# fjall-rs/lsm-tree

Measured on AMD Instinct MI355X. Metric: device-resident data-block decode+encode GiB/s, 1 M × 4 KiB blocks, higher is better.
Workload: dtype u8; 1 GPU; BASELINE configs[1]/[2]: encode + decode round trip of 1 M x 4 KiB data blocks, device-resident; blocks_per_gpu=1048576, items_per_gpu=54525952, block_bytes_per_gpu=3953267212, restart_interval=16, key_len=16, val_len=64, parallelism=shard1 (independent block batches, no collective)

## Files before the change

### lsm-tree_amd/csrc/encode_group.hpp

```cpp
#pragma once

#include "encode_plan.hpp"

namespace lsmgpu {

struct GBlk {
  uint32_t it0, n;
  uint32_t img, plen;
  uint32_t recs, bin_len;
  uint32_t step, hash_w;
  uint32_t hash_base, u0;
  uint32_t nbk, spare;
};
static_assert(sizeof(GBlk) == 48, "GBlk");

#ifdef LSM_NO_WAVE_BLOCKS
constexpr bool kWaveBlocks = false;
#else
constexpr bool kWaveBlocks = true;
#endif
constexpr uint32_t kWKeys = 1024, kWVals = 4096, kWImg = 4496;
constexpr uint32_t kWItems = kWave;
constexpr uint32_t kWUnits = 5;
static_assert((kWImg - 1) / 1024 <= 4 && (kWImg - 1) / 1024 + 1 <= kWUnits,
              "full KiB units and the tail unit of a payload");
constexpr uint32_t kWDefer = 4;
static_assert(kWDefer >= 1 && kWDefer <= kWave / 4, "one lane quad per deferred block");
static_assert(kWDefer * kWUnits * 8 * 8 <= kWImg, "the kept contributions fit the free image at the flush");
struct WaveSlot {
  uint8_t keys[kWKeys + kGSlack];
  uint8_t vals[kWVals + kGSlack];
  uint8_t img[kWImg + kGSlack];
  uint64_t contrib[kWUnits * 8];
};
static_assert(offsetof(WaveSlot, vals) % 16 == 0 && offsetof(WaveSlot, img) % 16 == 0 && sizeof(WaveSlot) % 16 == 0,
              "stage DMA and 16-B copy-out alignment");
constexpr uint32_t kGroupBody = kGKeys + kGVals + kGImg + 3 * kGSlack + kGUnion + 2 * kGBlocks * (uint32_t)sizeof(GBlk);
constexpr uint32_t kWaveSlots = kGWaves * (uint32_t)sizeof(WaveSlot);
constexpr uint32_t kWavePad = kWaveSlots > kGroupBody ? kWaveSlots - kGroupBody : 16;

struct GroupLds {
  uint8_t keys[kGKeys + kGSlack];
  uint8_t vals[kGVals + kGSlack];
  uint8_t img[kGImg + kGSlack];
  uint32_t uni[kGUnion / 4];
  GBlk blk[2][kGBlocks];
  uint8_t wave_pad[kWavePad];
  LongSecret secret;
};
static_assert(offsetof(GroupLds, uni) - offsetof(GroupLds, vals) >= sizeof(PlanWaveLds), "plan LDS over the stage");
static_assert(offsetof(GroupLds, vals) % 16 == 0, "plan LDS alignment");
static_assert(kGRunFused * (sizeof(BlockPlan) + 8) + 16 <= kGUnion, "fused plan outputs in uni");
static_assert(offsetof(GroupLds, wave_pad) == kGroupBody, "GroupLds layout");
static_assert(kGWaves * sizeof(WaveSlot) <= offsetof(GroupLds, secret), "the wave slots lie over the group loop's LDS");
static_assert(sizeof(GroupLds) <= 40960, "four workgroups per CU");

__device__ __host__ __forceinline__ bool wave_fits(uint64_t n, uint64_t kspan, uint64_t vspan, uint64_t total) {
  return n >= 1 && n <= kWItems && kspan + 15 <= kWKeys && vspan + 15 <= kWVals && total + 15 <= kWImg;
}


__device__ __forceinline__ void lds_copy(uint8_t* dst, uint32_t d, const uint8_t* src, uint32_t s, uint32_t n,
                                         uint32_t rot, uint32_t done = 0) {
  if (!n) return;
  const uint32_t h = min(n, (4u - (d & 3u)) & 3u);
  uint32_t hb[3];
#pragma unroll
  for (uint32_t k = 0; k < 3; ++k)
    if (k < h) hb[k] = src[s + k];
#pragma unroll
  for (uint32_t k = 0; k < 3; ++k)
    if (k < h) dst[d + k] = (uint8_t)hb[k];
  if (n == h) return;
  const uint32_t d1 = d + h + 4 * done, e = d + n, body = ((e & ~3u) - d1) >> 2;
  const uint32_t sp = s + h + 4 * done, sh = sp & 3u;
  const uint32_t* s32 = reinterpret_cast<const uint32_t*>(src + (sp & ~3u));
  uint32_t* d32 = reinterpret_cast<uint32_t*>(dst + d1);
  uint32_t q = ((rot & 31u) * body) >> 5;
  constexpr uint32_t U = 4;
  const uint32_t w0 = body ? s32[0] : 0;
  uint32_t carry = body ? s32[q] : 0;
  for (uint32_t j0 = 0; j0 < body; j0 += U) {
    uint32_t hi[U], at[U];
#pragma unroll
    for (uint32_t t = 0; t < U; ++t) {
      uint32_t p = q + t;
      p = p >= body ? p - body : p;
      at[t] = p;
      if (j0 + t < body) hi[t] = s32[p + 1];
    }
#pragma unroll
    for (uint32_t t = 0; t < U; ++t) {
      if (j0 + t < body) {
        const uint32_t lo = t == 0 ? carry : (at[t] == 0 ? w0 : hi[t - 1]);
        d32[at[t]] = alignbyte(hi[t], lo, sh);
      }
    }
    q += U;
    q = q >= body ? q - body : q;
    carry = q == 0 ? w0 : hi[U - 1];
  }
  const uint32_t t0 = d1 + 4 * body;
  uint32_t tb[3];
#pragma unroll
  for (uint32_t k = 0; k < 3; ++k)
    if (t0 + k < e) tb[k] = src[s + (t0 + k - d)];
#pragma unroll
  for (uint32_t k = 0; k < 3; ++k)
    if (t0 + k < e) dst[t0 + k] = (uint8_t)tb[k];
}

#ifdef LSM_NO_UNIFORM_COPY
constexpr bool kUniformCopy = false;
#else
constexpr bool kUniformCopy = true;
#endif
constexpr uint32_t kUniformMin = 4;
__device__ __forceinline__ uint32_t lds_copy_uniform(uint8_t* dst, uint32_t d, const uint8_t* src, uint32_t s,
                                                     uint32_t n, bool has, uint32_t rot) {
  if (!kUniformCopy) return 0;
  const uint32_t h = min(n, (4u - (d & 3u)) & 3u);
  const uint32_t body = n > h ? (((d + n) & ~3u) - (d + h)) >> 2 : 0u;
  const uint32_t B = wave_min_u32(has ? body : 0xFFFFFFFFu);
  if (B < kUniformMin || B == 0xFFFFFFFFu) return 0;
  if (has) {
    const uint8_t* sb = src + ((s + h) & ~3u);
    uint8_t* db = dst + d + h;
    const uint32_t sh = (s + h) & 3u, B4 = 4 * B;
    auto ld = [&](uint32_t x) { return *reinterpret_cast<const uint32_t*>(sb + x); };
    auto st = [&](uint32_t x, uint32_t v) { *reinterpret_cast<uint32_t*>(db + x) = v; };
    constexpr uint32_t U = kUniformMin;
    uint32_t x = (((rot & 31u) * B) >> 5) * 4;
    const uint32_t w0 = ld(0);
    uint32_t carry = ld(x);
    for (uint32_t j = 0; j < B; j += U) {
      uint32_t at[U], hi[U];
#pragma unroll
      for (uint32_t t = 0; t < U; ++t) {
        const uint32_t y = x + 4 * t;
        at[t] = t == 0 ? x : min(y, y - B4);
        hi[t] = ld(at[t] + 4);
      }
#pragma unroll
      for (uint32_t t = 0; t < U; ++t) {
        const uint32_t lo = at[t] == 0 ? w0 : (t == 0 ? carry : hi[t - 1]);
        st(at[t], alignbyte(hi[t], lo, sh));
      }
      carry = hi[U - 1];
      x += 4 * U;
      x = min(x, x - B4);
    }
    if (body > B) {
      st(B4, alignbyte(ld(B4 + 4), ld(B4), sh));
      return B + 1;
    }
  }
  return B;
}

__device__ __forceinline__ uint32_t lds_put_leb(uint8_t* dst, uint32_t pos, uint64_t v) {
  while (v >= 0x80) {
    dst[pos++] = (uint8_t)(v | 0x80);
    v >>= 7;
  }
  dst[pos++] = (uint8_t)v;
  return pos;
}

template <bool kIndex>
__device__ __forceinline__ uint32_t put_record_header(uint8_t* img, uint32_t pos, const uint8_t* keys, uint32_t kst,
                                                      const ItemMeta& m, bool head, uint32_t from, uint32_t rot) {
  if (kIndex) {
    img[pos++] = 0;
    pos = lds_put_leb(img, pos, m.vo);
    pos = lds_put_leb(img, pos, m.vl);
    pos = lds_put_leb(img, pos, m.seq);
    pos = lds_put_leb(img, pos, m.klen);
    lds_copy(img, pos, keys, kst, m.klen, rot);
  } else {
    img[pos++] = (uint8_t)m.vt;
    pos = lds_put_leb(img, pos, m.seq);
    if (!head) pos = lds_put_leb(img, pos, m.sh);
    pos = lds_put_leb(img, pos, m.klen - from);
    lds_copy(img, pos, keys, kst + from, m.klen - from, rot);
    pos += m.klen - from;
    if (!is_tombstone(m.vt)) pos = lds_put_leb(img, pos, m.vl);
  }
  return pos;
}

__device__ __forceinline__ void put_bin_entry(uint8_t* img, uint32_t bp, const uint32_t& step, uint32_t roff) {
  for (uint32_t q = 0; q < step; ++q) img[bp + q] = (uint8_t)(roff >> (8 * q));
}

__device__ __forceinline__ void group_barrier() {
  __builtin_amdgcn_fence(__ATOMIC_RELEASE, "workgroup", "local");
  __builtin_amdgcn_s_barrier();
  __builtin_amdgcn_fence(__ATOMIC_ACQUIRE, "workgroup", "local");
}

__device__ __forceinline__ void group_barrier_lds() {
  asm volatile("s_waitcnt lgkmcnt(0)\n\ts_barrier" ::: "memory");
}

#ifdef LSM_DIAG
#define ENC_PHASE(i)                                 \
  if (P.diag & kDiagGroupPhases) {                              \
    const uint64_t t_ = __builtin_amdgcn_s_memtime(); \
    ph_acc[i] += (uint32_t)(t_ - t_last);            \
    t_last = t_;                                     \
  }
#else
#define ENC_PHASE(i)
#endif

constexpr uint64_t kLbAgg = 1ULL << 62, kLbIncl = 2ULL << 62, kLbPoison = 1ULL << 61, kLbVal = kLbPoison - 1;
constexpr uint64_t kLookbackTicks = 10000000;

__device__ __forceinline__ uint64_t lb_load(const uint64_t* p) {
  return __hip_atomic_load(p, __ATOMIC_RELAXED, __HIP_MEMORY_SCOPE_AGENT);
}
__device__ __forceinline__ void lb_store(uint64_t* p, uint64_t v) {
  __hip_atomic_store(p, v, __ATOMIC_RELAXED, __HIP_MEMORY_SCOPE_AGENT);
}

__device__ __noinline__ uint64_t run_lookback(uint64_t* lb, uint32_t run, uint64_t agg, uint32_t diag, bool& poisoned) {
  const int lane = threadIdx.x & (kWave - 1);
  if (lane == 0) lb_store(lb + run, (run == 0 ? kLbIncl : kLbAgg) | agg);
  uint64_t excl = 0;
  bool poison = false;
  if (run != 0) {
    int64_t top = (int64_t)run - 1;
    uint64_t t0 = __builtin_amdgcn_s_memrealtime();
    for (;;) {
      const int64_t idx = top - lane;
      const uint64_t v = idx >= 0 ? lb_load(lb + idx) : kLbIncl;
      const uint64_t incl_m = __ballot((v >> 62) == 2), ready_m = __ballot((v >> 62) != 0);
      const uint32_t stop = incl_m ? (uint32_t)__builtin_ctzll(incl_m) : 64u;
      const uint64_t need = stop >= 63 ? ~0ULL : (2ULL << stop) - 1;
      if ((ready_m & need) == need && !(kDiagBuild && (diag & kDiagLookbackGiveUp))) {
        const bool mine = (uint32_t)lane <= stop;
        poison = poison || __ballot(mine && (v & kLbPoison)) != 0;
        excl += wave_bcast_u64(wave_incl_scan_u64(mine ? (v & kLbVal) : 0), kWave - 1);
        if (stop < 64) break;
        top -= 64;
        t0 = __builtin_amdgcn_s_memrealtime();
        continue;
      }
      if (__builtin_amdgcn_s_memrealtime() - t0 > kLookbackTicks || (kDiagBuild && (diag & kDiagLookbackGiveUp))) {
        poison = true;
        break;
      }
      __builtin_amdgcn_s_sleep(1);
    }
    if (lane == 0) lb_store(lb + run, kLbIncl | (poison ? kLbPoison : 0) | ((excl + agg) & kLbVal));
  }
  poisoned = poison;
  return excl;
}

__device__ __forceinline__ uint32_t lane_u32(uint32_t v, uint32_t l) {
  return (uint32_t)__shfl((int)v, (int)min(l, 63u));
}
__device__ __forceinline__ uint64_t lane_u64(uint64_t v, uint32_t l) { return wave_shfl_u64(v, (int)min(l, 63u)); }
__device__ __forceinline__ uint32_t rl32(uint32_t v, uint32_t l) {
  return (uint32_t)__builtin_amdgcn_readlane((int)v, (int)min(l, 63u));
}
__device__ __forceinline__ uint64_t rl64(uint64_t v, uint32_t l) {
  const int q = (int)min(l, 63u);
  return (uint64_t)(uint32_t)__builtin_amdgcn_readlane((int)(uint32_t)v, q) |
         ((uint64_t)(uint32_t)__builtin_amdgcn_readlane((int)(uint32_t)(v >> 32), q) << 32);
}
__device__ __forceinline__ uint32_t tpi_shift(uint32_t n) {
  return n <= kGThreads / 4 ? 2u : n <= kGThreads / 2 ? 1u : 0u;
}
template <bool kIndex, class Raw>
__device__ __forceinline__ ItemMeta cook_vetted(const Raw& r) {
  bool bad = false;
  return cook_item<kIndex>(r, bad);
}

template <bool kIndex, bool kHash, bool kPlanBkt, int kOW, bool kFused = false>
__global__ __launch_bounds__(kGThreads) __attribute__((amdgpu_waves_per_eu(4))) void encode_group_kernel(EncodeParams P) {
  static_assert(!kFused || (!kIndex && !kHash), "the fused plan is for data blocks without a hash index");
  __shared__ GroupLds L;
  const uint32_t tid = threadIdx.x;
  const uint32_t wave = __builtin_amdgcn_readfirstlane(tid / kWave);
  const int lane = tid & (kWave - 1);
  constexpr uint32_t kRun = kFused ? kGRunFused : kGRun;
  const uint32_t b_begin = blockIdx.x * kRun;
  const uint32_t b_end = min(b_begin + kRun, P.n_blocks);
  const uint32_t ri = kIndex ? 1 : P.ri;
  constexpr bool index = kIndex;
  if (tid < sizeof(LongSecret) / 8)
    reinterpret_cast<uint64_t*>(&L.secret)[tid] = reinterpret_cast<const uint64_t*>(&kLongSecret)[tid];
  const uint32_t rb = b_begin + lane;
  const bool in_run = rb <= b_end;
  const uint32_t r_start = in_run ? P.starts[rb] : 0;
  uint64_t r_off, r_ks, r_vs;
  BlockPlan r_plan;
  bool run_ok = true;
  if (kFused) {
    BlockPlan* const fplan = reinterpret_cast<BlockPlan*>(L.uni);
    uint64_t* const fsize = reinterpret_cast<uint64_t*>(L.uni) + 2 * kRun;
    uint64_t* const fbase = fsize + kRun;
    plan_wave_run<false, kOW, true>(P, b_begin, b_end - b_begin, *reinterpret_cast<PlanWaveLds*>(L.vals), fplan,
                                    fsize);
    __syncthreads();
    r_plan = rb < b_end ? fplan[lane] : BlockPlan{0, 0, 0, 0};
    const uint64_t sz = rb < b_end ? fsize[lane] : 0;
    const uint64_t incl = wave_incl_scan_u64(sz);
    if (wave == 0) {
      bool poisoned;
      const uint64_t base = run_lookback(P.sizes, blockIdx.x, wave_bcast_u64(incl, kWave - 1), P.diag, poisoned);
      if (lane == 0) {
        fbase[0] = base;
        fbase[1] = poisoned ? 1 : 0;
      }
    }
    __syncthreads();
    const uint64_t ex = fbase[0] + incl - sz;
    run_ok = fbase[1] == 0;
    r_off = in_run ? (ex & kOffMask) : 0;
    if (wave == 0 && rb < b_end) {
      P.block_off[rb] = r_off;
      if (!run_ok) P.status[rb] = ST_INCOMPLETE;
      else if (sz & ~kOffMask) P.lists[ex >> 40] = rb;
    }
    if (wave == 0 && rb == b_end && b_end == P.n_blocks) {
      P.block_off[rb] = r_off;
      P.list_count[0] = run_ok ? (uint32_t)(ex >> 40) : 0u;
    }
    const uint32_t cs = in_run ? clamped_start(P, rb) : 0;
    r_ks = in_run ? koff<kOW>(P, cs) : 0;
    r_vs = in_run ? voff<kOW>(P, cs) : 0;
    __syncthreads();
  } else {
    r_off = in_run ? P.block_off[rb] : 0;
    r_ks = in_run ? P.kspan[rb] : 0;
    r_vs = in_run ? P.vspan[rb] : 0;
    r_plan = (in_run && rb < b_end) ? P.plans[rb] : BlockPlan{0, 0, 0, 0};
  }
  const uint32_t r_hash = r_plan.hash_w;
  const uint32_t r_hpre = wave_incl_scan_u32(r_hash) - r_hash;
  uint32_t r_upre;
  {
    const uint64_t nx = wave_shfl_u64(r_off, min(lane + 1, 63));
    const uint32_t plen = (rb < b_end) ? (uint32_t)(nx - r_off) - kHdrLen : 0;
    const uint32_t units = plen > 240 ? (plen - 1) / 1024 + 1 : 0;
    r_upre = wave_incl_scan_u32(units) - units;
  }
  struct Grp {
    uint32_t b, k;
  };
  auto form = [&](uint32_t b) -> Grp {
    const uint32_t r0 = b - b_begin, rj = r0 + lane;
    const uint32_t s0 = rl32(r_start, r0), s1 = lane_u32(r_start, rj + 1);
    const uint64_t o0 = rl64(r_off, r0), o1 = lane_u64(r_off, rj + 1);
    const uint64_t k0 = rl64(r_ks, r0), k1 = lane_u64(r_ks, rj + 1);
    const uint64_t v0 = rl64(r_vs, r0), v1 = lane_u64(r_vs, rj + 1);
    const uint32_t flags = lane_u32(r_plan.step_flags, rj) >> 8;
    const uint32_t hsum = lane_u32(r_hpre, rj + 1) - rl32(r_hpre, r0);
    const bool ok = b + lane < b_end && lane < (int)kGBlocks && flags == 0 && o1 <= P.out_cap &&
                    group_fits(s1 - s0, k1 - (k0 & ~15ULL), v1 - (v0 & ~15ULL), o1 - (o0 & ~15ULL), hsum);
    return Grp{b, (uint32_t)__builtin_ctzll(~__ballot(ok))};
  };
  const uint64_t gmask = __ballot(rb < b_end && (r_plan.step_flags >> 8) == 0);
  auto next_group = [&](uint32_t b) -> Grp {
    for (;;) {
      if (b >= b_end) return Grp{b, 0};
      const Grp g = form(b);
      if (g.k) return g;
      const uint64_t rest = gmask >> (b - b_begin);
      if (rest & 1) {
        if (lane == 0) P.status[b] = ST_OVERFLOW;
        ++b;
      } else {
        b = rest ? b + (uint32_t)__builtin_ctzll(rest) : b_end;
      }
    }
  };
  auto issue_dma = [&](const Grp& g) {
    const uint32_t r0 = g.b - b_begin;
    const uint64_t ka = rl64(r_ks, r0) & ~15ULL, kb = rl64(r_ks, r0 + g.k);
    const uint64_t va = rl64(r_vs, r0) & ~15ULL, vb = rl64(r_vs, r0 + g.k);
    const uint32_t kc = (uint32_t)((kb - ka + 15) >> 4), vc = index ? 0 : (uint32_t)((vb - va + 15) >> 4);
    stage_to_lds(P.it.keys + ka, L.keys, kc, wave, kGWaves, lane);
    stage_to_lds(P.it.vals + va, L.vals, vc, wave, kGWaves, lane);
  };
  uint32_t* hlo = L.uni;
  uint32_t* hhi = hlo + kGHash;
  uint64_t* contrib = reinterpret_cast<uint64_t*>(L.uni);

  auto load_items = [&](const Grp& g, RawItemT<kOW, kIndex>& r) {
    const uint32_t r0 = g.b - b_begin;
    const uint32_t i0 = rl32(r_start, r0), n = rl32(r_start, r0 + g.k) - i0;
    const uint64_t i = (uint64_t)i0 + min(tid >> tpi_shift(n), n - 1);
    r = load_raw<kIndex, kOW>(P, i);
    r.e = P.erec[i];
    if (kPlanBkt) r.hb = P.hbucket[i];
  };

  auto build_table = [&](const Grp& g, GBlk* tb) {
    const uint32_t gr0 = g.b - b_begin, gk = g.k;
    const uint32_t gi0 = rl32(r_start, gr0);
    const uint64_t gob = rl64(r_off, gr0);
    const uint32_t gpad = (uint32_t)(((uint64_t)(uintptr_t)P.out + gob) & 15);
    const uint32_t rj = gr0 + lane;
    const uint32_t st = lane_u32(r_start, rj), st1 = lane_u32(r_start, rj + 1);
    const uint64_t of = lane_u64(r_off, rj), of1 = lane_u64(r_off, rj + 1);
    const uint32_t recs = lane_u32(r_plan.recs, rj), bin_len = lane_u32(r_plan.bin_len, rj);
    const uint32_t sf = lane_u32(r_plan.step_flags, rj), hw = lane_u32(r_plan.hash_w, rj);
    const uint32_t hb = lane_u32(r_hpre, rj) - rl32(r_hpre, gr0);
    const bool in = (uint32_t)lane < gk;
    const uint32_t plen = in ? (uint32_t)(of1 - of) - kHdrLen : 0;
    const uint32_t nbk = plen > 240 ? (plen - 1) / 1024 : 0;
    const uint32_t units = plen > 240 ? nbk + 1 : 0;
    const uint32_t u0 = wave_incl_scan_u32(units) - units;
    if (in) {
      GBlk B;
      B.it0 = st - gi0;
      B.n = st1 - st;
      B.img = (uint32_t)(of - gob) + gpad;
      B.plen = plen;
      B.recs = recs;
      B.bin_len = bin_len;
      B.step = sf & 0xFF;
      B.hash_w = hw;
      B.hash_base = hb;
      B.u0 = u0;
      B.nbk = nbk;
      B.spare = 0;
      tb[lane] = B;
    }
  };

  constexpr bool kWaveLoop = kWaveBlocks && !kIndex && !kHash && !kPlanBkt && !kFused;
  if constexpr (kWaveLoop) {
    bool wave_run;
    {
      const uint32_t s1 = lane_u32(r_start, lane + 1);
      const uint64_t o1 = lane_u64(r_off, lane + 1), k1 = lane_u64(r_ks, lane + 1), v1 = lane_u64(r_vs, lane + 1);
      const bool fit = (r_plan.step_flags >> 8) == 0 && o1 <= P.out_cap &&
                       wave_fits(s1 - r_start, k1 - (r_ks & ~15ULL), v1 - (r_vs & ~15ULL), o1 - (r_off & ~15ULL));
      wave_run = __ballot(rb < b_end && !fit) == 0 &&
                 !(kDiagBuild && (P.diag & (kDiagNoWaveBlocks | kDiagGroupLoopBits)));
    }
    if (wave_run) {
      WaveSlot& W = reinterpret_cast<WaveSlot*>(&L)[wave];
      auto wave_lds_wait = [&]() { asm volatile("s_waitcnt lgkmcnt(0)" ::: "memory"); };
      auto wave_dma = [&](uint32_t r) {
        const uint64_t ka = rl64(r_ks, r) & ~15ULL, kb = rl64(r_ks, r + 1);
        const uint64_t va = rl64(r_vs, r) & ~15ULL, vb = rl64(r_vs, r + 1);
        const uint32_t kc = (uint32_t)((kb - ka + 15) >> 4), vc = (uint32_t)((vb - va + 15) >> 4);
        stage_to_lds(P.it.keys + ka, W.keys, kc, 0, 1, lane);
        stage_to_lds(P.it.vals + va, W.vals, vc, 0, 1, lane);
      };
      auto wave_items = [&](uint32_t r, RawItemT<kOW, kIndex>& x) {
        const uint32_t i0 = rl32(r_start, r), n = rl32(r_start, r + 1) - i0;
        const uint64_t i = (uint64_t)i0 + min((uint32_t)lane, n - 1);
        x = load_raw<kIndex, kOW>(P, i);
        x.e = P.erec[i];
      };
      group_barrier_lds();
      uint32_t r = wave;
      const uint32_t nr = b_end - b_begin;
      RawItemT<kOW, kIndex> raw{};
      if (r < nr) {
        wave_dma(r);
        wave_items(r, raw);
      }
      vm_wait<0>();
      uint64_t d0 = 0, d1 = 0;
      uint64_t kc[kWDefer] = {};
      uint32_t dn = 0, dr = wave;
      auto flush_headers = [&]() {
        const uint32_t rj = dr + kGWaves * ((uint32_t)lane >> 2);
        const int q = lane & 3;
        const bool in = ((uint32_t)lane >> 2) < dn;
        const uint64_t ob = lane_u64(r_off, rj);
        const uint32_t plen = (uint32_t)(lane_u64(r_off, rj + 1) - ob) - kHdrLen;
        const bool lng = in && plen > 240;
        uint64_t lo = 0, hi = 0;
        constexpr uint32_t kCW = kWUnits * 8;
        uint64_t* const side = reinterpret_cast<uint64_t*>(W.img);
        if ((uint32_t)lane < kCW) {
#pragma unroll
          for (uint32_t s = 0; s < kWDefer; ++s) side[kCW * s + (uint32_t)lane] = kc[s];
        }
        wave_lds_wait();
        if (lng) {
          const uint32_t nbk = (plen - 1) / 1024;
          uint64_t a0, a1;
          xxh3_acc_init(q, a0, a1);
          const uint64_t scr0 = L.secret.acc[16 + 2 * q], scr1 = L.secret.acc[16 + 2 * q + 1];
          static_assert((kWImg - 1) / 1024 <= 4 && 4 <= kWUnits, "nbk <= 4: one batch is the whole chain");
          const uint64_t* cb = side + kCW * ((uint32_t)lane >> 2) + 2 * q;
          const uint64_t t0 = cb[8 * nbk], t1 = cb[8 * nbk + 1];
          xxh3_quad_chain_batch<4>(cb, 0, nbk, scr0, scr1, a0, a1);
          d0 = a0 + t0;
          d1 = a1 + t1;
        }
        if (lng) xxh3_merge_part(&L.secret, q, d0, d1, lo, hi);
        lo = quad_sum64(lo);
        hi = quad_sum64(hi);
        if (in) {
          if (lng) {
            xxh3_finish128(plen, lo, hi, lo, hi);
          } else {
            lo = d0;
            hi = d1;
          }
          write_header_quad((__attribute__((address_space(1))) uint8_t*)(P.out + ob), 0, P.type, lo, hi, plen, q);
          if (q == 0) P.status[b_begin + rj] = ST_OK;
        }
      };
      while (r < nr) {
        const uint32_t i0 = rl32(r_start, r), n = rl32(r_start, r + 1) - i0;
        const uint64_t kbase = rl64(r_ks, r) & ~15ULL, vbase = rl64(r_vs, r) & ~15ULL;
        const uint64_t obase = rl64(r_off, r);
        const uint32_t total = (uint32_t)(rl64(r_off, r + 1) - obase), plen = total - kHdrLen;
        const uint32_t recs = rl32(r_plan.recs, r), bin_len = rl32(r_plan.bin_len, r);
        const uint32_t step = rl32(r_plan.step_flags, r) & 0xFF;
        const uint64_t dabs = (uint64_t)(uintptr_t)P.out + obase;
        const uint32_t pad = (uint32_t)(dabs & 15), p0 = pad + kHdrLen;
        const uint32_t rn = r + kGWaves;
        const bool more = rn < nr;
        ItemMeta m = cook_vetted<kIndex>(raw);
        if (more) wave_items(rn, raw);
        {
          const bool live = (uint32_t)lane < n;
          const bool head = (m.e & kErecHead) != 0;
          m.sh = head ? 0u : m.e >> 16;
          const uint32_t roff = m.e & 0x7FFFu, from = head ? 0 : m.sh;
          const uint32_t kst = (uint32_t)(m.ko - kbase), vsrc = (uint32_t)(m.vo - vbase);
          const bool has_val = live && !is_tombstone(m.vt);
          uint32_t vpos = 0;
          if (live) vpos = put_record_header<false>(W.img, p0 + roff, W.keys, kst, m, head, from, lane);
          const uint32_t done = lds_copy_uniform(W.img, vpos, W.vals, vsrc, m.vl, has_val && m.vl != 0, lane);
          if (live) {
            if (has_val) lds_copy(W.img, vpos, W.vals, vsrc, m.vl, lane, done);
            if (head) put_bin_entry(W.img, p0 + recs + 1 + (m.e >> 16) * step, step, roff);
          }
        }
        if (lane == 0) W.img[p0 + recs] = kTrailerMarker;
        write_trailer_bytes(W.img, p0 + plen - kTrailerLen, ri, step, bin_len, recs + 1, 0, 0, n);
        wave_lds_wait();
        if (more) wave_dma(rn);
        if (plen > 240) {
          const uint32_t nbk = (plen - 1) / 1024;
          {
            const uint32_t row = (uint32_t)lane >> 4, rr = lane & 15;
            for (uint32_t u = row; u <= nbk; u += 4) {
              uint64_t c0, c1;
              xxh3_row_unit(W.img, p0, plen, nbk, u, rr, &L.secret, c0, c1);
              if (rr < 4) {
                W.contrib[8 * u + 2 * rr] = c0;
                W.contrib[8 * u + 2 * rr + 1] = c1;
              }
            }
          }
          wave_lds_wait();
          {
            const uint64_t cv = W.contrib[min((uint32_t)lane, kWUnits * 8 - 1)];
#pragma unroll
            for (uint32_t s = 0; s < kWDefer; ++s) kc[s] = dn == s ? cv : kc[s];
          }
        } else if (((uint32_t)lane >> 2) == dn) {
          xxh3_128_short(plen, BaseReader8{W.img, p0}, BaseReader64{W.img, p0}, d0, d1);
        }
        ++dn;
        vm_wait<0>();
        {
          const uint32_t end = pad + total, ch = (p0 + 15) >> 4, c1 = end >> 4;
          const u32x4* const csrc = reinterpret_cast<const u32x4*>(W.img);
          u32x4* const cdst = reinterpret_cast<u32x4*>(dabs & ~15ULL);
          for (uint32_t c = ch + (uint32_t)lane; c < c1; c += kWave)
            *(__attribute__((address_space(1))) u32x4*)(cdst + c) = csrc[c];
          auto* gb = (__attribute__((address_space(1))) uint8_t*)cdst;
          const uint32_t x = (uint32_t)lane;
          if (p0 + x < min(16 * ch, end)) gb[p0 + x] = W.img[p0 + x];
          if (c1 >= ch && 16 * c1 + x < end) gb[16 * c1 + x] = W.img[16 * c1 + x];
        }
        wave_lds_wait();
        if (dn == kWDefer || !more) {
          flush_headers();
          dn = 0;
          dr = rn;
        }
        r = rn;
      }
      return;
    }
  }

#ifdef LSM_DIAG
  uint64_t t_last = __builtin_amdgcn_s_memtime();
  uint32_t ph_acc[12] = {};
  uint32_t ph_n = 0;
#endif
  Grp G = run_ok ? next_group(b_begin) : Grp{b_end, 0};
  RawItemT<kOW, kIndex> raw{};
  if (G.k) {
    issue_dma(G);
    load_items(G, raw);
    if (wave == 0) build_table(G, L.blk[0]);
  }
  vm_lgkm_wait0();
  ENC_PHASE(11);
  uint32_t iter = 0;
  while (G.k) {
    ENC_PHASE(0);
    const uint32_t r0 = G.b - b_begin, k = G.k;
    const uint32_t i0 = rl32(r_start, r0), n_items = rl32(r_start, r0 + k) - i0;
    const uint64_t kbase = rl64(r_ks, r0) & ~15ULL, vbase = rl64(r_vs, r0) & ~15ULL;
    const uint64_t obase = rl64(r_off, r0);
    const uint64_t dabs = (uint64_t)(uintptr_t)P.out + obase;
    const uint32_t pad = (uint32_t)(dabs & 15);
    const uint32_t tsh = tpi_shift(n_items), part = tid & ((1u << tsh) - 1), item = tid >> tsh;
    const bool live = item < n_items;
    const Grp Gn = next_group(G.b + k);
    ItemMeta m = cook_vetted<kIndex>(raw);
    if (Gn.k) load_items(Gn, raw);
    ENC_PHASE(9);
    GBlk* const TB = L.blk[iter & 1];
    const uint32_t hsum = rl32(r_hpre, r0 + k) - rl32(r_hpre, r0);
    for (uint32_t h = tid; h < hsum; h += kGThreads) {
      hlo[h] = 0xFFFFFFFFu;
      hhi[h] = 0;
    }
    group_barrier_lds();
    ENC_PHASE(1);
    uint32_t j = 0;
    for (uint32_t jb = 1; jb < k; ++jb) j += (rl32(r_start, r0 + jb) - i0 <= item) ? 1u : 0u;
    const bool head = (m.e & kErecHead) != 0;
    m.sh = head ? 0u : m.e >> 16;
    const bool writes = live && !(kDiagBuild && (P.diag & (kDiagNoRecordStores | kDiagNoRecordsTails)));
    const uint32_t roff = m.e & 0x7FFFu;
    const uint32_t from = head ? 0 : m.sh;
    const uint32_t kst = (uint32_t)(m.ko - kbase);
    const bool has_val = writes && !index && !is_tombstone(m.vt);
    const uint32_t vsrc = (uint32_t)(m.vo - vbase);
    auto put_header = [&]() -> uint32_t {
      return put_record_header<index>(L.img, TB[j].img + kHdrLen + roff, L.keys, kst, m, head, from, lane);
    };
    auto put_index_and_vote = [&]() {
      const GBlk& B = TB[j];
      if (head) put_bin_entry(L.img, B.img + kHdrLen + B.recs + 1 + (m.e >> 16) * B.step, B.step, roff);
      if (kHash && B.hash_w) {
        const uint32_t ridx = (item - B.it0) / ri;
        const uint32_t hb =
            kPlanBkt ? m.hb
                     : (uint32_t)(xxh3_64_any(m.klen, BaseReader8{L.keys, kst}, BaseReader64{L.keys, kst}) % B.hash_w);
        const uint32_t bk = B.hash_base + hb;
        atomicMin(&hlo[bk], ridx);
        atomicMax(&hhi[bk], ridx);
      }
    };
    constexpr bool uniform = !index;
    if (tsh == 0) {
      uint32_t vpos = 0;
      if (writes) vpos = put_header();
      const uint32_t done =
          uniform ? lds_copy_uniform(L.img, vpos, L.vals, vsrc, m.vl, has_val && m.vl != 0, lane) : 0u;
      if (writes) {
        if (has_val) lds_copy(L.img, vpos, L.vals, vsrc, m.vl, lane, done);
        put_index_and_vote();
      }
    } else {
      const uint32_t va = (part * m.vl) >> tsh, vb = ((part + 1) * m.vl) >> tsh;
      uint32_t vpos = 0;
      if (writes) {
        if (part == 0)
          vpos = put_header();
        else if (has_val)
          vpos = TB[j].img + kHdrLen + roff + 1 + leb_len(m.seq) + (head ? 0u : leb_len(m.sh)) + leb_len(m.klen - from) +
                 (m.klen - from) + leb_len(m.vl);
      }
      const uint32_t done =
          uniform ? lds_copy_uniform(L.img, vpos + va, L.vals, vsrc + va, vb - va, has_val && vb != va, lane) : 0u;
      if (writes) {
        if (has_val) lds_copy(L.img, vpos + va, L.vals, vsrc + va, vb - va, lane, done);
        if (part == 0) put_index_and_vote();
      }
    }
    auto tails = [&]() {
      for (uint32_t jb = wave; jb < (kDiagBuild && (P.diag & kDiagNoRecordsTails) ? 0 : k); jb += kGWaves) {
        const GBlk& B = TB[jb];
        const uint32_t p0 = B.img + kHdrLen, bin_off = B.recs + 1;
        if (lane == 0) L.img[p0 + B.recs] = kTrailerMarker;
        const uint32_t hash_off = B.hash_w ? bin_off + B.bin_len * B.step : 0;
        if (kHash)
          for (uint32_t q = lane; q < B.hash_w; q += kWave)
            L.img[p0 + hash_off + q] = (uint8_t)bucket_byte(hlo[B.hash_base + q], hhi[B.hash_base + q]);
        write_trailer_bytes(L.img, p0 + B.plen - kTrailerLen, ri, B.step, B.bin_len, bin_off, B.hash_w, hash_off,
                            B.n);
      }
    };
    if (!kHash) tails();
    group_barrier_lds();
    ENC_PHASE(3);
    if (Gn.k && !(kDiagBuild && (P.diag & kDiagNoNextDma))) issue_dma(Gn);
    ENC_PHASE(10);
    if (kHash) {
      tails();
      group_barrier_lds();
    }
    ENC_PHASE(4);
    {
      const uint32_t row = wave * 4 + (lane >> 4), r = lane & 15, q = r & 3;
      const uint32_t ubase = rl32(r_upre, r0);
      const uint32_t units =
          (kDiagBuild && (P.diag & (kDiagNoHash | kDiagNoRecordsTails))) ? 0 : rl32(r_upre, r0 + k) - ubase;
      for (uint32_t u = row; u < units; u += 4 * kGWaves) {
        uint32_t jb = 0;
        for (uint32_t x = 1; x < k; ++x) jb += (rl32(r_upre, r0 + x) - ubase <= u) ? 1u : 0u;
        const GBlk& B = TB[jb];
        uint64_t c0, c1;
        xxh3_row_unit(L.img, B.img + kHdrLen, B.plen, B.nbk, u - B.u0, r, &L.secret, c0, c1);
        if (r < 4) {
          contrib[8 * u + 2 * q] = c0;
          contrib[8 * u + 2 * q + 1] = c1;
        }
      }
    }
    group_barrier_lds();
    ENC_PHASE(5);
    const uint32_t cw = iter & (kGWaves - 1);
    const uint32_t total = (uint32_t)(rl64(r_off, r0 + k) - obase);
    const uint32_t end = (kDiagBuild && (P.diag & kDiagNoCopyOut)) ? pad : pad + total;
    const uint32_t c0 = (pad + 15) >> 4, c1 = end >> 4;
    const u32x4* const csrc = reinterpret_cast<const u32x4*>(L.img);
    u32x4* const cdst = reinterpret_cast<u32x4*>(dabs & ~15ULL);
    const uint32_t hpc = (wave == cw && (uint32_t)lane < 3 * k) ? (TB[lane / 3].img >> 4) + lane % 3 : ~0u;
    if (wave == cw) {
      if (!(kDiagBuild && (P.diag & (kDiagNoHash | kDiagNoRecordsTails)))) {
        const uint32_t jb = (uint32_t)lane >> 2;
        const int q = lane & 3;
        const bool in = jb < k;
        const GBlk& B = TB[in ? jb : 0];
        const uint32_t p0 = B.img + kHdrLen, plen = B.plen;
        uint64_t lo = 0, hi = 0;
        if (in && plen > 240) {
          uint64_t a0, a1;
          xxh3_acc_init(q, a0, a1);
          const uint64_t scr0 = L.secret.acc[16 + 2 * q], scr1 = L.secret.acc[16 + 2 * q + 1];
          const uint64_t* cb = contrib + 8 * B.u0 + 2 * q;
          xxh3_quad_chain<4>(cb, B.nbk, scr0, scr1, a0, a1);
          a0 += cb[8 * B.nbk];
          a1 += cb[8 * B.nbk + 1];
          xxh3_merge_part(&L.secret, q, a0, a1, lo, hi);
        }
        lo = quad_sum64(lo);
        hi = quad_sum64(hi);
        if (in) {
          if (plen > 240) {
            xxh3_finish128(plen, lo, hi, lo, hi);
          } else {
            xxh3_128_short(plen, BaseReader8{L.img, p0}, BaseReader64{L.img, p0}, lo, hi);
          }
          write_header_quad(L.img, B.img, P.type, lo, hi, plen, q);
          if (q == 0) P.status[G.b + jb] = ST_OK;
        }
      }
    } else {
      if (Gn.k && wave == ((cw + 1) & (kGWaves - 1))) build_table(Gn, L.blk[(iter + 1) & 1]);
      const uint32_t t3 = ((wave + kGWaves - cw - 1) & (kGWaves - 1)) * kWave + (uint32_t)lane;
      constexpr uint32_t kT3 = (kGWaves - 1) * kWave;
      uint32_t hc = __builtin_amdgcn_readfirstlane(TB[0].img) >> 4;
      for (uint32_t jb = 0; jb < k; ++jb) {
        const uint32_t hn = jb + 1 < k ? __builtin_amdgcn_readfirstlane(TB[jb + 1].img) >> 4 : c1;
        for (uint32_t c = max(hc + 3, c0) + t3; c < min(hn, c1); c += kT3)
          *(__attribute__((address_space(1))) u32x4*)(cdst + c) = csrc[c];
        hc = hn;
      }
    }
    group_barrier_lds();
    ENC_PHASE(6);
    vm_lgkm_wait0();
    ENC_PHASE(7);
    {
      if (hpc >= c0 && hpc < c1) *(__attribute__((address_space(1))) u32x4*)(cdst + hpc) = csrc[hpc];
      auto* gb = (__attribute__((address_space(1))) uint8_t*)cdst;
      if (tid == 0)
        for (uint32_t x = pad; x < min(16 * c0, end); ++x) gb[x] = L.img[x];
      if (tid == kWave && c1 >= c0)
        for (uint32_t x = 16 * c1; x < end; ++x) gb[x] = L.img[x];
    }
    ENC_PHASE(8);
#ifdef LSM_DIAG
    ++ph_n;
#endif
    ++iter;
    G = Gn;
  }
#ifdef LSM_DIAG
  if ((P.diag & kDiagGroupPhases) && tid == 0) {
    for (int i = 0; i < 12; ++i) atomicAdd(&P.phase[i], (unsigned long long)ph_acc[i]);
    atomicAdd(&P.phase[15], (unsigned long long)ph_n);
  }
#endif
}

extern template __global__ void encode_group_kernel<false, true, false, 4, false>(EncodeParams);
extern template __global__ void encode_group_kernel<false, true, false, 8, false>(EncodeParams);

}
```

### lsm-tree_amd/csrc/encode_plan.hpp

```cpp
#pragma once

#include "encode_common.hpp"

namespace lsmgpu {

__device__ __forceinline__ uint64_t e2_need(uint64_t total, uint32_t hash_w) {
  return ((15 + total + 15) & ~15ULL) + 32 + 8ULL * ((hash_w + 3) & ~3u);
}

template <bool kIndex>
__device__ __forceinline__ uint64_t plan_block(const EncodeParams& P, uint32_t b, uint32_t s, uint32_t e, bool bad,
                                               uint64_t recs, uint64_t last_head, uint64_t ks, uint64_t ke,
                                               uint64_t vs, uint64_t ve, BlockPlan& pl) {
  const uint32_t ri = kIndex ? 1 : P.ri;
  const uint32_t n = bad ? 0 : e - s;
  if (bad) recs = last_head = 0;
  const uint32_t bin_len = n ? (n + ri - 1) / ri : 0;
  const uint32_t step = last_head <= 0xFFFF ? 2 : 4;
  const uint32_t buckets = kIndex ? 0 : bucket_count(n, P.ratio);
  const uint32_t hash_w = (buckets > 0 && bin_len <= kHashMaxPointers) ? buckets : 0;
  const uint64_t total = kHdrLen + recs + 1 + (uint64_t)bin_len * step + hash_w + kTrailerLen;
  if (recs > 0xFFFFFFF0ULL || total > 0xFFFFFF00ULL) bad = true;
  uint32_t flags = 0;
  if (bad) {
    flags = kPlanBad;
    P.status[b] = ST_BAD_ARG;
  } else if (!group_fits(n, ke - ks, ve - vs, total, hash_w)) {
    const uint64_t need = e2_need(total, hash_w);
    flags = need <= kImgMedium ? kPlanMedium : need <= kImgBig ? kPlanBig : kPlanHuge;
  }
  pl = BlockPlan{(uint32_t)recs, bin_len, hash_w, step | (flags << 8)};
  P.plans[b] = pl;
  return (bad ? 0 : total) | ((flags & (kPlanMedium | kPlanBig | kPlanHuge)) ? kListedOne : 0);
}

__device__ __forceinline__ Win16 gwin16(const uint8_t* p) {
  Win16 r;
  __builtin_memcpy(&r, p, 16);
  return r;
}
__device__ __forceinline__ Win16 gwin16a(const uint8_t* p) { return gwin16(p); }

__device__ __noinline__
uint32_t lcp_tail(const uint8_t* keys, uint64_t a, uint64_t b, uint32_t n) {
  for (uint32_t k = 16; k < n; k += 16) {
    const Win16 wa = gwin16(keys + a + k), wb = gwin16(keys + b + k);
    const uint64_t x0 = wa.lo ^ wb.lo, x1 = wa.hi ^ wb.hi;
    if (x0) return min(n, k + (uint32_t)(__builtin_ctzll(x0) >> 3));
    if (x1) return min(n, k + 8 + (uint32_t)(__builtin_ctzll(x1) >> 3));
  }
  return n;
}

constexpr uint32_t kPW = 2;
constexpr uint32_t kPWStep = kPW * kWave;
struct PlanWaveLds {
  uint32_t bst[kPlanBlocks + 1];
  uint32_t badf[kPlanBlocks];
  uint32_t wcut[5];
  uint32_t mono;
  unsigned long long bfirst[kPlanBlocks], bend[kPlanBlocks], lhead[kPlanBlocks];
  unsigned long long kos[4][kPWStep];
  uint32_t kls[4][kPWStep];
  Win16 kwin[4][kPWStep];
};

template <bool kBkt, int kOW, bool kFused>
__device__ __forceinline__ void plan_wave_run(const EncodeParams& P, uint32_t b0, uint32_t nb, PlanWaveLds& S,
                                              BlockPlan* fplan, uint64_t* fsize) {
  uint32_t* const bst = S.bst;
  unsigned long long* const bfirst = S.bfirst;
  unsigned long long* const bend = S.bend;
  unsigned long long* const lhead = S.lhead;
  auto& kos = S.kos;
  auto& kls = S.kls;
  auto& kwin = S.kwin;
  uint32_t* const badf = S.badf;
  uint32_t* const wcut = S.wcut;
  uint32_t& mono = S.mono;
  const uint32_t tid = threadIdx.x, lane = tid & (kWave - 1);
  const uint32_t wave = __builtin_amdgcn_readfirstlane(tid / kWave);
  if (tid <= nb) bst[tid] = clamped_start(P, b0 + tid);
  if (tid < nb) {
    bfirst[tid] = bend[tid] = lhead[tid] = 0;
    badf[tid] = 0;
  }
  if (tid == 0) mono = 1;
  __syncthreads();
  if (tid < nb && bst[tid + 1] < bst[tid]) mono = 0;
  if (tid <= 4) {
    const uint32_t target = bst[0] + (uint32_t)(((uint64_t)(bst[nb] - bst[0]) * tid) / 4);
    uint32_t lo = 0, hi = nb;
    while (lo < hi) {
      const uint32_t mid = (lo + hi) >> 1;
      if (bst[mid] >= target) hi = mid;
      else lo = mid + 1;
    }
    wcut[tid] = tid == 4 ? nb : lo;
  }
  __syncthreads();
  const uint32_t ri = P.ri;
  const uint32_t jlo = __builtin_amdgcn_readfirstlane(wcut[wave]);
  const uint32_t jhi = __builtin_amdgcn_readfirstlane(mono ? wcut[wave + 1] : wcut[wave]);
  const uint32_t ia = __builtin_amdgcn_readfirstlane(bst[jlo]);
  const uint32_t ie = __builtin_amdgcn_readfirstlane(bst[jhi]);
  unsigned long long* wkos = kos[wave];
  uint32_t* wkls = kls[wave];
  Win16* wkwin = kwin[wave];
  struct StepRaw {
    typename RawItemT<kOW>::off_t ko[kPW + 1], vo[kPW + 1];
    uint64_t seq[kPW];
    uint32_t vt[kPW];
  };
  auto load_step = [&](uint32_t base, StepRaw& r) {
    const uint32_t n = ie - base, t = min(kPW * lane, n - 1);
    auto at64 = [&](const uint64_t* a, uint32_t k) {
      return *reinterpret_cast<const uint64_t*>(reinterpret_cast<const uint8_t*>(a + base) + 8u * k);
    };
#pragma unroll
    for (uint32_t q = 0; q <= kPW; ++q) {
      r.ko[q] = (typename RawItemT<kOW>::off_t)off_rel<kOW>(P, P.it.key_off, base, min(t + q, n));
      r.vo[q] = (typename RawItemT<kOW>::off_t)off_rel<kOW>(P, P.it.val_off, base, min(t + q, n));
    }
#pragma unroll
    for (uint32_t q = 0; q < kPW; ++q) {
      r.seq[q] = at64(P.it.seqno, min(t + q, n - 1));
      r.vt[q] = (P.it.vtype + base)[min(t + q, n - 1)];
    }
  };
  StepRaw raw;
  if (ia < ie) load_step(ia, raw);
  uint64_t carry = 0;
  uint64_t hk_ko = 0;
  uint32_t hk_kl = 0;
  Win16 hk_win{0, 0};
  for (uint32_t base = ia; base < ie; base += kPWStep) {
    const uint32_t t0 = kPW * lane;
    ItemMeta m[kPW];
    uint32_t jq[kPW], jjq[kPW];
    bool ok[kPW];
    uint32_t j = jlo;
    {
      uint32_t lo = jlo, hi = jhi;
      const uint32_t i0 = min(base + t0, ie - 1);
      while (hi - lo > 1) {
        const uint32_t mid = (lo + hi) >> 1;
        if (bst[mid] <= i0) lo = mid;
        else hi = mid;
      }
      j = lo;
    }
#pragma unroll
    for (uint32_t q = 0; q < kPW; ++q) {
      const uint32_t i = base + t0 + q;
      ok[q] = i < ie;
      while (j + 1 < jhi && bst[j + 1] <= i) ++j;
      jq[q] = j;
      jjq[q] = ok[q] ? i - bst[j] : 0;
      bool bad = false;
      RawItem r;
      r.ko = raw.ko[q];
      r.ko1 = raw.ko[q + 1];
      r.vo = raw.vo[q];
      r.vo1 = raw.vo[q + 1];
      r.seq = raw.seq[q];
      r.vt = raw.vt[q];
      r.e = 0;
      r.hb = kNoBucket;
      m[q] = cook_item<false>(r, bad);
      if (ok[q] && bad) atomicOr(&badf[j], 1u);
      wkos[t0 + q] = m[q].ko;
      wkls[t0 + q] = m[q].klen;
    }
    if (base + kPWStep < ie) load_step(base + kPWStep, raw);
    Win16 wa[kPW], wb[kPW];
#pragma unroll
    for (uint32_t q = 0; q < kPW; ++q) wb[q] = gwin16a(P.it.keys + m[q].ko);
#pragma unroll
    for (uint32_t q = 0; q < kPW; ++q) wkwin[t0 + q] = wb[q];
    if (kBkt) {
#pragma unroll
      for (uint32_t q = 0; q < kPW; ++q) {
        if (!ok[q]) continue;
        const uint32_t n = bst[jq[q] + 1] - bst[jq[q]];
        const uint32_t buckets = bucket_count(n, P.ratio);
        const uint32_t hw = (buckets > 0 && (n + ri - 1) / ri <= kHashMaxPointers) ? buckets : 0;
        uint32_t hb = kNoBucket;
        if (hw && hw < kNeedHash) {
          if (m[q].klen <= 16)
            hb = (uint32_t)(xxh3_64_le16(m[q].klen, WinReader8{wb[q].lo, wb[q].hi},
                                         WinReader64{wb[q].lo, wb[q].hi}) % hw);
          else
            hb = kNeedHash, P.hb_fix[0] = 1;
        }
        P.hbucket[(uint64_t)base + t0 + q] = (uint16_t)hb;
      }
    }
    wave_lds_sync();
    uint32_t nq[kPW];
    uint64_t hq[kPW];
#pragma unroll
    for (uint32_t q = 0; q < kPW; ++q) {
      nq[q] = 0;
      hq[q] = 0;
      wa[q] = wb[q];
      if (ok[q] && jjq[q] % ri != 0) {
        const uint32_t h = base + t0 + q - jjq[q] % ri;
        const bool in = h >= base;
        const uint64_t hko = in ? (uint64_t)wkos[h - base] : hk_ko;
        const uint32_t hkl = in ? wkls[h - base] : hk_kl;
        nq[q] = min(hkl, m[q].klen);
        hq[q] = hko;
        wa[q] = in ? wkwin[h - base] : hk_win;
      }
    }
#pragma unroll
    for (uint32_t q = 0; q < kPW; ++q) {
      if (!nq[q]) continue;
      const uint64_t x0 = wa[q].lo ^ wb[q].lo, x1 = wa[q].hi ^ wb[q].hi;
      const uint32_t n = nq[q];
      uint32_t sh;
      if (x0) sh = min(n, (uint32_t)(__builtin_ctzll(x0) >> 3));
      else if (x1) sh = min(n, 8 + (uint32_t)(__builtin_ctzll(x1) >> 3));
      else sh = n <= 16 ? n : lcp_tail(P.it.keys, hq[q], m[q].ko, n);
      m[q].sh = sh;
    }
    uint64_t rec[kPW], tsum = 0;
#pragma unroll
    for (uint32_t q = 0; q < kPW; ++q) {
      rec[q] = ok[q] ? item_record_len(P, m[q], jjq[q] % ri == 0) : 0;
      tsum += rec[q];
    }
    const uint64_t incl = wave_incl_scan_u64(tsum);
    uint64_t ex = carry + incl - tsum;
    uint64_t exq[kPW];
#pragma unroll
    for (uint32_t q = 0; q < kPW; ++q) {
      exq[q] = ex;
      if (ok[q]) {
        const uint32_t jb = jq[q], jj = jjq[q], ridx = jj / ri;
        const uint32_t n = bst[jb + 1] - bst[jb];
        if (jj == 0) bfirst[jb] = ex;
        if (jj + 1 == n) bend[jb] = ex + rec[q];
        if (jj == ridx * ri && ridx == (n - 1) / ri) lhead[jb] = ex;
      }
      ex += rec[q];
    }
    wave_lds_sync();
#pragma unroll
    for (uint32_t q = 0; q < kPW; ++q) {
      if (ok[q]) {
        const uint32_t jj = jjq[q], ridx = jj / ri;
        const bool head = jj == ridx * ri;
        const uint64_t roff = exq[q] - bfirst[jq[q]];
        const uint32_t x = head ? ridx : m[q].sh;
        P.erec[(uint64_t)base + t0 + q] =
            bst[jq[q] + 1] - bst[jq[q]] > kGItems
                ? (uint32_t)min(roff, (uint64_t)0xFFFFFFFFu)
                : (uint32_t)min(roff, (uint64_t)0x7FFF) | (head ? kErecHead : 0u) | (min(x, 0xFFFFu) << 16);
      }
    }
    carry += wave_bcast_u64(incl, kWave - 1);
    {
      const uint32_t last = min(ie, base + kPWStep) - 1, ll = (last - base) / kPW, lq = (last - base) % kPW;
      uint32_t jsel = jjq[0];
#pragma unroll
      for (uint32_t q = 1; q < kPW; ++q) jsel = lq == q ? jjq[q] : jsel;
      const uint32_t jjl = __builtin_amdgcn_readlane((int)jsel, (int)ll);
      const uint32_t h = last - jjl % ri;
      if (h >= base) {
        hk_ko = wkos[h - base];
        hk_kl = wkls[h - base];
        hk_win = wkwin[h - base];
      }
    }
    wave_lds_sync();
  }
  __syncthreads();
  if (tid >= nb) return;
  const uint32_t b = b0 + tid, s = bst[tid], e = bst[tid + 1];
  const bool bad = !mono || e <= s || badf[tid] || start_past_items(P, b + 1);
  const uint64_t ks = koff<kOW>(P, s), ke = koff<kOW>(P, e);
  const uint64_t vs = voff<kOW>(P, s), ve = voff<kOW>(P, e);
  BlockPlan pl;
  const uint64_t size =
      plan_block<false>(P, b, s, e, bad, bend[tid] - bfirst[tid], lhead[tid] - bfirst[tid], ks, ke, vs, ve, pl);
  if (kFused) {
    fplan[tid] = pl;
    fsize[tid] = size;
    if (size & ~kOffMask) P.status[b] = ST_INCOMPLETE;
  } else {
    P.sizes[b] = size;
  }
  P.kspan[b] = ks;
  P.vspan[b] = vs;
  if (b + 1 == P.n_blocks) {
    P.kspan[b + 1] = ke;
    P.vspan[b + 1] = ve;
  }
}

}
```

Measured before the change: 1028 GiB/s.

## Add quick register-only block planner and enable wave loop in fused path

Adds a fast per-wave planning path for fused runs where every block holds at most one wave's worth of items. Each wave plans several blocks entirely in registers: prefix lengths via key windows, record sizes via a wave scan, and erec writes, replacing the general LDS-based plan_wave_run. It also lets the fused kernel take the wave-blocks encode loop, gated on run_ok, and computes key and value spans before planning. This adds code paths and register pressure, and the fallback to the general planner stays in place.

```diff
diff --git a/lsm-tree_amd/csrc/encode_group.hpp b/lsm-tree_amd/csrc/encode_group.hpp
--- a/lsm-tree_amd/csrc/encode_group.hpp
+++ b/lsm-tree_amd/csrc/encode_group.hpp
@@ -21,6 +21,7 @@
 #endif
 constexpr uint32_t kWKeys = 1024, kWVals = 4096, kWImg = 4496;
 constexpr uint32_t kWItems = kWave;
+static_assert(kQItems == kWItems, "the quick plan sizes what this loop writes");
 constexpr uint32_t kWUnits = 5;
 static_assert((kWImg - 1) / 1024 <= 4 && (kWImg - 1) / 1024 + 1 <= kWUnits,
               "full KiB units and the tail unit of a payload");
@@ -304,8 +305,16 @@
     BlockPlan* const fplan = reinterpret_cast<BlockPlan*>(L.uni);
     uint64_t* const fsize = reinterpret_cast<uint64_t*>(L.uni) + 2 * kRun;
     uint64_t* const fbase = fsize + kRun;
-    plan_wave_run<false, kOW, true>(P, b_begin, b_end - b_begin, *reinterpret_cast<PlanWaveLds*>(L.vals), fplan,
-                                    fsize);
+    const uint32_t cs = in_run ? ((uint64_t)r_start > P.it.n_items ? (uint32_t)P.it.n_items : r_start) : 0;
+    r_ks = in_run ? koff<kOW>(P, cs) : 0;
+    r_vs = in_run ? voff<kOW>(P, cs) : 0;
+    const uint32_t cs_next = lane_u32(cs, lane + 1);
+    const bool quick = kQuickPlan && P.it.n_items != 0 && __ballot(rb < b_end && cs_next - cs > kQItems) == 0;
+    if (quick)
+      plan_quick_run<kOW>(P, b_begin, b_end - b_begin, r_start, cs, fplan, fsize);
+    else
+      plan_wave_run<false, kOW, true>(P, b_begin, b_end - b_begin, *reinterpret_cast<PlanWaveLds*>(L.vals), fplan,
+                                      fsize);
     __syncthreads();
     r_plan = rb < b_end ? fplan[lane] : BlockPlan{0, 0, 0, 0};
     const uint64_t sz = rb < b_end ? fsize[lane] : 0;
@@ -331,9 +340,6 @@
       P.block_off[rb] = r_off;
       P.list_count[0] = run_ok ? (uint32_t)(ex >> 40) : 0u;
     }
-    const uint32_t cs = in_run ? clamped_start(P, rb) : 0;
-    r_ks = in_run ? koff<kOW>(P, cs) : 0;
-    r_vs = in_run ? voff<kOW>(P, cs) : 0;
     __syncthreads();
   } else {
     r_off = in_run ? P.block_off[rb] : 0;
@@ -435,7 +441,8 @@
     }
   };
 
-  constexpr bool kWaveLoop = kWaveBlocks && !kIndex && !kHash && !kPlanBkt && !kFused;
+  constexpr bool kWaveLoop = kWaveBlocks && !kIndex && !kHash && !kPlanBkt;
+  constexpr uint32_t kDiagOffWave = (kFused ? 0u : kDiagNoWaveBlocks) | kDiagGroupLoopBits;
   if constexpr (kWaveLoop) {
     bool wave_run;
     {
@@ -443,8 +450,7 @@
       const uint64_t o1 = lane_u64(r_off, lane + 1), k1 = lane_u64(r_ks, lane + 1), v1 = lane_u64(r_vs, lane + 1);
       const bool fit = (r_plan.step_flags >> 8) == 0 && o1 <= P.out_cap &&
                        wave_fits(s1 - r_start, k1 - (r_ks & ~15ULL), v1 - (r_vs & ~15ULL), o1 - (r_off & ~15ULL));
-      wave_run = __ballot(rb < b_end && !fit) == 0 &&
-                 !(kDiagBuild && (P.diag & (kDiagNoWaveBlocks | kDiagGroupLoopBits)));
+      wave_run = run_ok && __ballot(rb < b_end && !fit) == 0 && !(kDiagBuild && (P.diag & kDiagOffWave));
     }
     if (wave_run) {
       WaveSlot& W = reinterpret_cast<WaveSlot*>(&L)[wave];
diff --git a/lsm-tree_amd/csrc/encode_plan.hpp b/lsm-tree_amd/csrc/encode_plan.hpp
--- a/lsm-tree_amd/csrc/encode_plan.hpp
+++ b/lsm-tree_amd/csrc/encode_plan.hpp
@@ -300,4 +300,144 @@
   }
 }
 
-}
+#ifdef LSM_NO_QUICK_PLAN
+constexpr bool kQuickPlan = false;
+#else
+constexpr bool kQuickPlan = true;
+#endif
+constexpr uint32_t kQItems = kWave;
+constexpr uint32_t kQBlocks = (kGRunFused + kGWaves - 1) / kGWaves;
+
+__device__ __forceinline__ uint32_t readlane_off(uint32_t v, uint32_t l) { return wave_readlane_u32(v, l); }
+__device__ __forceinline__ uint64_t readlane_off(uint64_t v, uint32_t l) { return wave_readlane_u64(v, l); }
+__device__ __forceinline__ uint32_t shfl_off(uint32_t v, uint32_t l) { return wave_bcast_u32(v, (int)l); }
+__device__ __forceinline__ uint64_t shfl_off(uint64_t v, uint32_t l) { return wave_shfl_u64(v, (int)l); }
+
+template <int kOW>
+__device__ __forceinline__ void plan_quick_run(const EncodeParams& P, uint32_t b0, uint32_t nb, uint32_t r_start,
+                                               uint32_t cs, BlockPlan* fplan, uint64_t* fsize) {
+  typedef typename RawItemT<kOW>::off_t off_t;
+  constexpr uint32_t kQ = kQBlocks;
+  const uint32_t lane = threadIdx.x & (kWave - 1);
+  const uint32_t wave = __builtin_amdgcn_readfirstlane(threadIdx.x / kWave);
+  const uint32_t ri = P.ri;
+  const uint32_t ridx = lane / ri, hl = ridx * ri;
+  const bool head = hl == lane;
+  uint32_t s[kQ], n[kQ];
+  bool bad[kQ];
+  RawItemT<kOW> raw[kQ];
+#pragma unroll
+  for (uint32_t k = 0; k < kQ; ++k) {
+    const uint32_t j = wave + kGWaves * k;
+    const uint32_t jc = j < nb ? j : 0;
+    s[k] = wave_readlane_u32(cs, jc);
+    n[k] = j < nb ? wave_readlane_u32(cs, jc + 1) - s[k] : 0;
+    bad[k] = n[k] == 0 || (uint64_t)wave_readlane_u32(r_start, jc + 1) > P.it.n_items;
+    const uint32_t sl = bad[k] ? 0 : s[k], t = bad[k] ? 0 : min(lane, n[k] - 1);
+    raw[k].ko = (off_t)off_rel<kOW>(P, P.it.key_off, sl, t);
+    raw[k].ko1 = (off_t)off_rel<kOW>(P, P.it.key_off, sl, t + 1);
+    raw[k].vo = (off_t)off_rel<kOW>(P, P.it.val_off, sl, t);
+    raw[k].vo1 = (off_t)off_rel<kOW>(P, P.it.val_off, sl, t + 1);
+    raw[k].seq = *reinterpret_cast<const uint64_t*>(reinterpret_cast<const uint8_t*>(P.it.seqno + sl) + 8u * t);
+    raw[k].vt = (P.it.vtype + sl)[t];
+    raw[k].e = 0;
+    raw[k].hb = kNoBucket;
+  }
+  __builtin_amdgcn_sched_barrier(0);
+  off_t ko[kQ];
+  uint32_t klen[kQ], ksp[kQ], vsp[kQ];
+  uint64_t rech[kQ];
+#pragma unroll
+  for (uint32_t k = 0; k < kQ; ++k) {
+    bool b = false;
+    const ItemMeta m = cook_item<false>(raw[k], b);
+    ko[k] = raw[k].ko;
+    klen[k] = m.klen;
+    rech[k] = item_record_len(P, m, true);
+    const uint32_t last = bad[k] ? 0 : n[k] - 1;
+    ksp[k] = (uint32_t)min((uint64_t)readlane_off(raw[k].ko1, last) - (uint64_t)readlane_off(raw[k].ko, 0),
+                           (uint64_t)0xFFFFFFFFu);
+    vsp[k] = (uint32_t)min((uint64_t)readlane_off(raw[k].vo1, last) - (uint64_t)readlane_off(raw[k].vo, 0),
+                           (uint64_t)0xFFFFFFFFu);
+    const bool item_bad = __ballot(lane < n[k] && b) != 0;
+    bad[k] = bad[k] || item_bad;
+  }
+  Win16 win[kQ];
+#pragma unroll
+  for (uint32_t k = 0; k < kQ; ++k) {
+    win[k] = Win16{0, 0};
+    if (!bad[k]) win[k] = gwin16(P.it.keys + ko[k]);
+  }
+  __builtin_amdgcn_sched_barrier(0);
+  uint32_t sh[kQ];
+  uint64_t rec[kQ], incl[kQ];
+#pragma unroll
+  for (uint32_t k = 0; k < kQ; ++k) {
+    sh[k] = 0;
+    rec[k] = 0;
+    if (!bad[k]) {
+      const uint32_t hkl = wave_bcast_u32(klen[k], (int)hl);
+      const uint64_t hko = shfl_off(ko[k], hl);
+      const Win16 wa{wave_shfl_u64(win[k].lo, (int)hl), wave_shfl_u64(win[k].hi, (int)hl)};
+      const bool live = lane < n[k];
+      if (live && !head) {
+        const uint32_t nn = min(hkl, klen[k]);
+        const uint64_t x0 = wa.lo ^ win[k].lo, x1 = wa.hi ^ win[k].hi;
+        uint32_t v;
+        if (x0) v = min(nn, (uint32_t)(__builtin_ctzll(x0) >> 3));
+        else if (x1) v = min(nn, 8 + (uint32_t)(__builtin_ctzll(x1) >> 3));
+        else v = nn <= 16 ? nn : lcp_tail(P.it.keys, hko, ko[k], nn);
+        sh[k] = v;
+      }
+      if (live)
+        rec[k] = head ? rech[k]
+                      : rech[k] - leb_len(klen[k]) + leb_len(sh[k]) + leb_len(klen[k] - sh[k]) - sh[k];
+    }
+    incl[k] = rec[k];
+  }
+#pragma unroll
+  for (int d = 1; d < (int)kWave; d <<= 1) {
+#pragma unroll
+    for (uint32_t k = 0; k < kQ; ++k) {
+      const uint32_t lo = __shfl_up((int)(uint32_t)incl[k], d), hi = __shfl_up((int)(uint32_t)(incl[k] >> 32), d);
+      if ((int)lane >= d) incl[k] += (uint64_t)lo | ((uint64_t)hi << 32);
+    }
+  }
+  uint32_t p_s = 0, p_n = 0, p_ks = 0, p_vs = 0;
+  uint64_t p_recs = 0, p_lhead = 0;
+  bool p_bad = true;
+#pragma unroll
+  for (uint32_t k = 0; k < kQ; ++k) {
+    uint64_t recs = 0, lhead = 0;
+    if (!bad[k]) {
+      const bool live = lane < n[k];
+      const uint64_t ex = incl[k] - rec[k];
+      recs = wave_readlane_u64(incl[k], kWave - 1);
+      const uint64_t heads = __ballot(live && head);
+      lhead = wave_readlane_u64(ex, 63u - (uint32_t)__builtin_clzll(heads));
+      if (live)
+        P.erec[(uint64_t)s[k] + lane] = (uint32_t)min(ex, (uint64_t)0x7FFF) | (head ? kErecHead : 0u) |
+                                        (min(head ? ridx : sh[k], 0xFFFFu) << 16);
+    }
+    if (lane == k) {
+      p_s = s[k];
+      p_n = n[k];
+      p_ks = ksp[k];
+      p_vs = vsp[k];
+      p_recs = recs;
+      p_lhead = lhead;
+      p_bad = bad[k];
+    }
+  }
+  const uint32_t j = wave + kGWaves * lane;
+  if (lane < kQ && j < nb) {
+    const uint32_t b = b0 + j;
+    BlockPlan pl;
+    const uint64_t size = plan_block<false>(P, b, p_s, p_s + p_n, p_bad, p_recs, p_lhead, 0, p_ks, 0, p_vs, pl);
+    fplan[j] = pl;
+    fsize[j] = size;
+    if (size & ~kOffMask) P.status[b] = ST_INCOMPLETE;
+  }
+}
+
+}
```

Result: no change. 1026 GiB/s, median of 3 (-0.2%).
